# ilur98/DLMC-QUANT

Measured on NVIDIA B200. Metric: fakequant_fwd_bwd_hbm_gbps, higher is better.
Workload: dtype f32

## Files before the change

dlmc_quant_b200/csrc/fq_kernels.cu:

```cuda
#include <mutex>

#include "fq_rows.cuh"

namespace dlmcq {

constexpr int kUnroll = 4;

template <int FORM, typename T, int U = kUnroll, int MINB = 4, bool TILED = false>
__global__ void __launch_bounds__(kThreads, MINB)
fq_fwd_flat(const T* __restrict__ x, T* __restrict__ y, T* __restrict__ codes, int64_t n,
            const float* __restrict__ scale, const float* __restrict__ offset, float g, float lo, float hi,
            int independent) {
  using V = Vec<T>;
  using raw = typename V::raw;
  const int64_t nvec = n / V::N;
  const raw* xv = reinterpret_cast<const raw*>(x);
  const int64_t tile_vecs = static_cast<int64_t>(U) * blockDim.x;
  const int64_t ntiles = nvec / tile_vecs;
  ChanParams p;
  raw r0[U];
  const bool hoist = TILED && independent && blockIdx.x < ntiles;
  if (TILED && independent) {
    p = make_params<FORM>(scale, offset, 0, g, lo, hi);
    if (hoist) {
      const int64_t b = static_cast<int64_t>(blockIdx.x) * tile_vecs + threadIdx.x;
#pragma unroll
      for (int k = 0; k < U; ++k) r0[k] = ld_stream(xv + b + k * blockDim.x);
    }
  }
  pdl_wait();
  pdl_trigger();
  if (!(TILED && independent)) p = make_params<FORM>(scale, offset, 0, g, lo, hi);
  const int64_t stride = static_cast<int64_t>(gridDim.x) * blockDim.x;
  int64_t i = static_cast<int64_t>(blockIdx.x) * blockDim.x + threadIdx.x;
  raw* yv = reinterpret_cast<raw*>(y);
  raw* cv = reinterpret_cast<raw*>(codes);

  auto body = [&](const raw& r, int64_t idx) {
    float f[V::N], fy[V::N], fc[V::N];
// ... 53 lines not shown
    if (codes) codes[i] = from_f32<T>(c);
  }
}

template <int FORM>
__device__ __forceinline__ void finalize_flat(float* partials, int nblocks, float g, float* dscale, float* doffset,
                                              float* smem) {
  double s = 0.0, o = 0.0;
  for (int b = threadIdx.x; b < nblocks; b += blockDim.x) {
    s += static_cast<double>(partials[2 * b]);
    o += static_cast<double>(partials[2 * b + 1]);
  }
  s = warp_sum(s);
  o = warp_sum(o);
  double* sm = reinterpret_cast<double*>(smem);
  const int lane = threadIdx.x & 31, warp = threadIdx.x >> 5, nwarp = blockDim.x >> 5;
  __syncthreads();
  if (lane == 0) { sm[warp] = s; sm[32 + warp] = o; }
  __syncthreads();
  if (threadIdx.x == 0) {
    double ts = 0.0, to = 0.0;
    for (int w = 0; w < nwarp; ++w) { ts += sm[w]; to += sm[32 + w]; }
    float r = static_cast<float>(ts);
    if (FORM == DLMCQ_FORM_AFFINE || FORM == DLMCQ_FORM_A1) r = r * g;
    dscale[0] = r;
    if (doffset) doffset[0] = static_cast<float>(to);
  }
}

template <int FORM, typename T, bool VECTOR, bool WANT_OFF, bool DEFER>
__global__ void __launch_bounds__(kThreads, 4)
fq_bwd_flat(const T* __restrict__ x, const T* __restrict__ dy, T* __restrict__ dx, int64_t n,
            const float* __restrict__ scale, const float* __restrict__ offset, float g, float lo, float hi,
            float* __restrict__ dscale, float* __restrict__ doffset, void* ws, int independent) {
  using V = Vec<T>;
  using raw = typename V::raw;
  __shared__ __align__(16) float smem[128];
  const int64_t nvec = n / V::N;
  const raw* xv = reinterpret_cast<const raw*>(x);
  const raw* gv = reinterpret_cast<const raw*>(dy);
  const int64_t tile_vecs = static_cast<int64_t>(kUnroll) * blockDim.x;
  const int64_t ntiles = nvec / tile_vecs;
  ChanParams p;
  raw rx0[kUnroll], rg0[kUnroll];
  const bool hoist = VECTOR && independent && blockIdx.x < ntiles;
  if (VECTOR && independent) {
    p = make_params<FORM>(scale, offset, 0, g, lo, hi);
    if (hoist) {
      const int64_t b = static_cast<int64_t>(blockIdx.x) * tile_vecs + threadIdx.x;
#pragma unroll
      for (int k = 0; k < kUnroll; ++k) {
        rx0[k] = ld_stream(xv + b + k * blockDim.x);
        rg0[k] = ld_stream(gv + b + k * blockDim.x);
      }
    }
  }
  pdl_wait();
  pdl_trigger();
  if (!(VECTOR && independent)) p = make_params<FORM>(scale, offset, 0, g, lo, hi);
  float acc[2] = {0.f, 0.f};
  const int64_t stride = static_cast<int64_t>(gridDim.x) * blockDim.x;
  int64_t i = static_cast<int64_t>(blockIdx.x) * blockDim.x + threadIdx.x;
  if (VECTOR) {
    raw* ov = reinterpret_cast<raw*>(dx);
    auto body = [&](const raw& rx, const raw& rg, int64_t idx) {
      float fx[V::N], fg[V::N], fo[V::N];
      V::unpack(rx, fx);
      V::unpack(rg, fg);
      fq_vec_bwd<FORM, WANT_OFF, V::N>(fx, fg, p, lo, hi, fo, acc[0], acc[1]);
      st_stream(ov + idx, V::pack(fo));
    };
    int64_t t = blockIdx.x;
    if (hoist) {
      const int64_t b = t * tile_vecs + threadIdx.x;
#pragma unroll
      for (int k = 0; k < kUnroll; ++k) body(rx0[k], rg0[k], b + k * blockDim.x);
      t += gridDim.x;
    }
    for (; t < ntiles; t += gridDim.x) {
      const int64_t b = t * tile_vecs + threadIdx.x;
      raw rx[kUnroll], rg[kUnroll];
#pragma unroll
      for (int k = 0; k < kUnroll; ++k) {
        rx[k] = ld_stream(xv + b + k * blockDim.x);
        rg[k] = ld_stream(gv + b + k * blockDim.x);
      }
#pragma unroll
      for (int k = 0; k < kUnroll; ++k) body(rx[k], rg[k], b + k * blockDim.x);
    }
    for (int64_t j = ntiles * tile_vecs + i; j < nvec; j += stride) body(ld_stream(xv + j), ld_stream(gv + j), j);
    if (blockIdx.x == 0) {
      const int64_t t = nvec * V::N + threadIdx.x;
      if (t < n) dx[t] = from_f32<T>(fq_elem_bwd<FORM, WANT_OFF>(to_f32<T>(x[t]), to_f32<T>(dy[t]), p, lo, hi, acc[0], acc[1]));
    }
  } else {
    for (; i < n; i += stride)
      dx[i] = from_f32<T>(fq_elem_bwd<FORM, WANT_OFF>(to_f32<T>(x[i]), to_f32<T>(dy[i]), p, lo, hi, acc[0], acc[1]));
  }
  block_sum<2>(acc, smem);
  if (DEFER) {
    float* out = static_cast<float*>(ws);
    if (threadIdx.x == 0) {
      if (blockIdx.x == 0) {
        out[0] = __int_as_float(static_cast<int>(gridDim.x));
        out[1] = (FORM == DLMCQ_FORM_AFFINE || FORM == DLMCQ_FORM_A1) ? g : 1.f;
      }
      out[2 + 2 * blockIdx.x] = acc[0];
      out[3 + 2 * blockIdx.x] = acc[1];
    }
    return;
  }
  float* partials = ws_partials(ws);
  if (threadIdx.x == 0) {
    partials[2 * blockIdx.x] = acc[0];
    partials[2 * blockIdx.x + 1] = acc[1];
  }
  if (take_last_ticket(ws_counter(ws), gridDim.x)) {
    finalize_flat<FORM>(partials, gridDim.x, g, dscale, doffset, smem);
    if (threadIdx.x == 0) *ws_counter(ws) = 0u;
  }
}

template <int FORM, typename T>
__global__ void __launch_bounds__(kRowWarps * 32, 3)
fq_fwd_rows(const T* __restrict__ x, T* __restrict__ y, T* __restrict__ codes, RowGeom gm,
            const float* __restrict__ scale, const float* __restrict__ offset, float g, float lo, float hi) {
  const int lane = threadIdx.x & 31;
  const int64_t item = static_cast<int64_t>(blockIdx.x) * kRowWarps + (threadIdx.x >> 5);
  if (item >= gm.rows * gm.segs) return;
  const int64_t row = item / gm.segs, seg = item - row * gm.segs;
// ... 456 lines not shown
    fq_slab_kernel<FORM, T><<<static_cast<unsigned>(sg.groups) * sg.chunks, kThreads, 0, st>>>(
        static_cast<const T*>(x), static_cast<T*>(y), static_cast<T*>(codes), sg, qp->scale, qp->offset, qp->g, lo, hi);
  } else if (cmaj_ok(l->outer, l->channels, l->inner)) {
    const bool vec = cmaj_vec_ok<T>(l->inner, x, y, codes, nullptr);
    const CmajGeom cg = make_cmaj(l->outer, l->channels, l->inner, vec ? Vec<T>::N : 1);
    const int64_t blocks = (cg.channels * cg.chunks + kRowWarps - 1) / kRowWarps;
    if (blocks > 0x7fffffffLL) return DLMCQ_EUNSUPPORTED;
    auto kern = vec ? fq_cmaj_kernel<FORM, T, false, Vec<T>::N> : fq_cmaj_kernel<FORM, T, false, 1>;
    kern<<<static_cast<unsigned>(blocks), kRowWarps * 32, 0, st>>>(
        static_cast<const T*>(x), nullptr, static_cast<T*>(y), static_cast<T*>(codes), cg, qp->scale, qp->offset,
        qp->g, lo, hi, nullptr, nullptr, 0);
  } else {
    const RowGeom gm = make_geom(l);
    const int64_t items = gm.rows * gm.segs;
    const int64_t blocks = (items + kRowWarps - 1) / kRowWarps;
    if (blocks > 0x7fffffffLL) return DLMCQ_EUNSUPPORTED;
    fq_fwd_rows<FORM, T><<<static_cast<unsigned>(blocks), kRowWarps * 32, 0, st>>>(
        static_cast<const T*>(x), static_cast<T*>(y), static_cast<T*>(codes), gm, qp->scale, qp->offset, qp->g, lo, hi);
  }
  DLMCQ_LAUNCH_CHECK();
  return DLMCQ_OK;
}

template <int FORM, typename T>
static int launch_bwd(const void* x, const void* dy, void* dx, float* dscale, float* doffset, const dlmcq_layout* l,
                      const dlmcq_qparams* qp, void* ws, size_t ws_bytes, cudaStream_t st, bool defer = false) {
  const int64_t n = l->outer * l->channels * l->inner;
  const float lo = static_cast<float>(qp->lo), hi = static_cast<float>(qp->hi);
  if (!defer && ws_bytes < dlmcq_workspace_bytes(l)) return DLMCQ_EWORKSPACE;
  if (defer && l->channels != 1) return DLMCQ_EUNSUPPORTED;
  if (l->channels == 1) {
    const bool vec = aligned16(x) && aligned16(dy) && aligned16(dx);
    const int64_t per = vec ? Vec<T>::N : 1;
    int64_t tiles = (n / per + kThreads * kUnroll - 1) / (kThreads * kUnroll);
    int64_t cap = n < (int64_t(1) << 25) ? 888 : (n < (int64_t(1) << 27) ? 2048 : 4096);
    if (cap > kMaxPartialBlocks) cap = kMaxPartialBlocks;
    const int grid = static_cast<int>(tiles < 1 ? 1 : (tiles < cap ? tiles : cap));
    auto k = vec ? (doffset ? fq_bwd_flat<FORM, T, true, true, false> : fq_bwd_flat<FORM, T, true, false, false>)
                 : (doffset ? fq_bwd_flat<FORM, T, false, true, false> : fq_bwd_flat<FORM, T, false, false, false>);
    if (defer) k = vec ? fq_bwd_flat<FORM, T, true, false, true> : fq_bwd_flat<FORM, T, false, false, true>;
    FlatAccess acc;
    if (vec) {
      const size_t bytes = static_cast<size_t>(n) * sizeof(T);
      acc.read(x, bytes);
      acc.read(dy, bytes);
      acc.read(qp->scale, sizeof(float));
      acc.read(qp->offset, sizeof(float));
      if (!defer) acc.read(ws, ws_bytes);
      acc.write(dx, bytes);
      acc.write(dscale, sizeof(float));
      acc.write(doffset, sizeof(float));
      acc.write(ws, defer ? (2 + 2 * static_cast<size_t>(grid)) * sizeof(float) : ws_bytes);
    }
    const int independent = vec ? capture_check(st, acc) : 0;
    cudaError_t e = launch_pdl(k, dim3(grid), dim3(kThreads), 0, st, static_cast<const T*>(x),
                               static_cast<const T*>(dy), static_cast<T*>(dx), n, qp->scale, qp->offset, qp->g, lo, hi,
                               dscale, doffset, ws, independent);
    if (e != cudaSuccess) return set_cuda_error(e);
    if (vec) capture_record(st, acc, independent);
  } else if (doffset == nullptr && n > 0 && tiled_ok<T>(l, x, dy, dx)) {
    const TileGeom tg = make_tile_geom<T>(l);
    const int64_t tiles = (tg.nvec + kTileVecs - 1) / kTileVecs;
    if (tiles > 0x7fffffffLL) return DLMCQ_EUNSUPPORTED;
    fq_tiled_chan_kernel<FORM, T, true><<<static_cast<unsigned>(tiles), kThreads, 0, st>>>(
        static_cast<const T*>(x), static_cast<const T*>(dy), static_cast<T*>(dx), nullptr, tg, qp->scale, qp->offset,
        qp->g, lo, hi, ws_partials(ws));
    DLMCQ_LAUNCH_CHECK();
    const float gmul = (FORM == DLMCQ_FORM_AFFINE || FORM == DLMCQ_FORM_A1) ? qp->g : 1.f;
    tiled_chan_finalize<<<static_cast<unsigned>(l->channels), 128, 0, st>>>(ws_partials(ws), tg, l->outer, gmul, dscale);
  } else if (cmaj_ok(l->outer, l->channels, l->inner) && doffset == nullptr && n > 0) {
    const bool vec = cmaj_vec_ok<T>(l->inner, x, dy, dx, nullptr);
    const CmajGeom cg = make_cmaj(l->outer, l->channels, l->inner, vec ? Vec<T>::N : 1);
    const int64_t blocks = (cg.channels * cg.chunks + kRowWarps - 1) / kRowWarps;
    if (blocks > 0x7fffffffLL) return DLMCQ_EUNSUPPORTED;
    const int direct = cg.chunks == 1 ? 1 : 0;
    auto kern = vec ? fq_cmaj_kernel<FORM, T, true, Vec<T>::N> : fq_cmaj_kernel<FORM, T, true, 1>;
    kern<<<static_cast<unsigned>(blocks), kRowWarps * 32, 0, st>>>(
        static_cast<const T*>(x), static_cast<const T*>(dy), static_cast<T*>(dx), nullptr, cg, qp->scale, qp->offset,
        qp->g, lo, hi, dscale, ws_partials(ws), direct);
    if (!direct) {
      DLMCQ_LAUNCH_CHECK();
      const float gmul = (FORM == DLMCQ_FORM_AFFINE || FORM == DLMCQ_FORM_A1) ? qp->g : 1.f;
      chan_finalize<1><<<static_cast<unsigned>(cg.channels), 128, 0, st>>>(ws_partials(ws), cg.chunks, cg.chunks, 0,
                                                                           gmul, dscale, nullptr);
    }
  } else {
    const RowGeom gm = make_geom(l);
    const int64_t items = gm.rows * gm.segs;
    const int64_t blocks = (items + kRowWarps - 1) / kRowWarps;
    if (blocks > 0x7fffffffLL) return DLMCQ_EUNSUPPORTED;
// ... 8 lines not shown
      chan_finalize<2><<<static_cast<unsigned>(gm.channels), 128, 0, st>>>(
          ws_partials(ws), l->outer * gm.segs, gm.segs, gm.channels * gm.segs, gmul, dscale, doffset);
    }
  }
  DLMCQ_LAUNCH_CHECK();
  return DLMCQ_OK;
}

template <typename T>
static int dispatch_fwd(const void* x, void* y, void* codes, const dlmcq_layout* l, const dlmcq_qparams* qp,
                        cudaStream_t st) {
  switch (qp->form) {
    case DLMCQ_FORM_A1: return launch_fwd<DLMCQ_FORM_A1, T>(x, y, codes, l, qp, st);
    case DLMCQ_FORM_AFFINE: return launch_fwd<DLMCQ_FORM_AFFINE, T>(x, y, codes, l, qp, st);
    case DLMCQ_FORM_ZP: return launch_fwd<DLMCQ_FORM_ZP, T>(x, y, codes, l, qp, st);
    case DLMCQ_FORM_SYM: return launch_fwd<DLMCQ_FORM_SYM, T>(x, y, codes, l, qp, st);
  }
  return DLMCQ_EINVAL;
}
template <typename T>
static int dispatch_bwd(const void* x, const void* dy, void* dx, float* ds, float* doff, const dlmcq_layout* l,
                        const dlmcq_qparams* qp, void* ws, size_t wsb, cudaStream_t st, bool defer = false) {
  switch (qp->form) {
    case DLMCQ_FORM_A1: return launch_bwd<DLMCQ_FORM_A1, T>(x, dy, dx, ds, doff, l, qp, ws, wsb, st, defer);
    case DLMCQ_FORM_AFFINE: return launch_bwd<DLMCQ_FORM_AFFINE, T>(x, dy, dx, ds, doff, l, qp, ws, wsb, st, defer);
    case DLMCQ_FORM_ZP: return launch_bwd<DLMCQ_FORM_ZP, T>(x, dy, dx, ds, doff, l, qp, ws, wsb, st, defer);
    case DLMCQ_FORM_SYM: return launch_bwd<DLMCQ_FORM_SYM, T>(x, dy, dx, ds, doff, l, qp, ws, wsb, st, defer);
  }
  return DLMCQ_EINVAL;
}

__global__ void __launch_bounds__(kThreads)
finalize_many_kernel(const dlmcq_finalize_item* __restrict__ items, int n_items) {
  __shared__ double sm[2][kThreads / 32];
  pdl_wait();
  pdl_trigger();
  const dlmcq_finalize_item it = items[blockIdx.x];
  const float* p = it.partials;
  const int nblocks = __float_as_int(p[0]);
  const float gmul = p[1];
  double s = 0.0, o = 0.0;
  for (int b = threadIdx.x; b < nblocks; b += blockDim.x) {
    s += static_cast<double>(p[2 + 2 * b]);
    o += static_cast<double>(p[3 + 2 * b]);
  }
  s = warp_sum(s);
  o = warp_sum(o);
  const int lane = threadIdx.x & 31, warp = threadIdx.x >> 5;
  if (lane == 0) { sm[0][warp] = s; sm[1][warp] = o; }
  __syncthreads();
  if (threadIdx.x == 0) {
    double ts = 0.0, to = 0.0;
    for (int w = 0; w < kThreads / 32; ++w) { ts += sm[0][w]; to += sm[1][w]; }
    it.dscale[0] = static_cast<float>(ts) * gmul;
    (void)to;
  }
}

}

using namespace dlmcq;

extern "C" size_t dlmcq_workspace_bytes(const dlmcq_layout* l) {
  size_t bytes = kWsHeaderBytes + static_cast<size_t>(kMaxPartialBlocks) * 96 * sizeof(float);
  if (l && l->outer >= 1 && l->channels >= 1 && l->inner >= 0) {
    const RowGeom gm = make_geom(l->outer, l->channels, l->inner);
    const size_t rows_bytes = static_cast<size_t>(gm.rows * gm.segs) * 4 * sizeof(float);
    if (kWsHeaderBytes + rows_bytes > bytes) bytes = kWsHeaderBytes + rows_bytes;
    const size_t tiles = static_cast<size_t>(l->outer * l->channels * l->inner) / (kTileVecs * 4) + 1;
    const size_t tiled_bytes = tiles * kTileRows * sizeof(float);
    if (kWsHeaderBytes + tiled_bytes > bytes) bytes = kWsHeaderBytes + tiled_bytes;
  }
  return bytes;
}

extern "C" int dlmcq_fq_forward(const void* x, void* y, void* codes, const dlmcq_layout* layout,
                                const dlmcq_qparams* qp, void* stream) {
  if (int e = check_layout(layout)) return e;
  if (layout->outer * layout->channels * layout->inner == 0) return DLMCQ_OK;
  if (!qp || !qp->scale || !x || (!y && !codes)) return DLMCQ_EINVAL;
  if (!elem_aligned(x, layout->dtype) || !elem_aligned(y, layout->dtype) || !elem_aligned(codes, layout->dtype))
    return DLMCQ_EALIGN;
  cudaStream_t st = static_cast<cudaStream_t>(stream);
  return layout->dtype == DLMCQ_F32 ? dispatch_fwd<float>(x, y, codes, layout, qp, st)
                                    : dispatch_fwd<__nv_bfloat16>(x, y, codes, layout, qp, st);
}

extern "C" int dlmcq_fq_backward(const void* x, const void* dy, void* dx, float* dscale, float* doffset,
// ... 62 lines not shown
```

dlmc_quant_b200/csrc/grouped_kernels.cu:

```cuda
#include "fq_rows.cuh"

namespace dlmcq {

__device__ __forceinline__ int find_item(const int64_t* __restrict__ prefix, int n_items, int64_t unit) {
  int lo = 0, hi = n_items;
  while (hi - lo > 1) {
    const int mid = (lo + hi) >> 1;
    if (__ldg(prefix + mid) <= unit) lo = mid; else hi = mid;
  }
  return lo;
}

template <int FORM>
__device__ __forceinline__ ChanParams item_params(const dlmcq_group_item& it, int64_t ch) {
  return make_params<FORM>(it.scale, it.offset, ch, it.g, static_cast<float>(it.lo), static_cast<float>(it.hi));
}

template <typename T>
__global__ void __launch_bounds__(kRowWarps * 32)
grouped_fwd_kernel(const dlmcq_group_item* __restrict__ items, const int64_t* __restrict__ prefix, int n_items,
                   int64_t total_units) {
  pdl_wait();
  pdl_trigger();
  const int lane = threadIdx.x & 31;
  const int64_t unit = static_cast<int64_t>(blockIdx.x) * kRowWarps + (threadIdx.x >> 5);
  if (unit >= total_units) return;
  const int k = find_item(prefix, n_items, unit);
  const dlmcq_group_item it = items[k];
  const int64_t local = unit - __ldg(prefix + k);
  const int64_t segs = (it.inner + DLMCQ_GROUP_SEG - 1) / DLMCQ_GROUP_SEG;
  const int64_t row = local / segs, seg = local - row * segs;
  const int64_t beg = seg * DLMCQ_GROUP_SEG;
  const int64_t len = (it.inner - beg) < DLMCQ_GROUP_SEG ? (it.inner - beg) : DLMCQ_GROUP_SEG;
  const T* xr = static_cast<const T*>(it.x) + row * it.inner + beg;
  T* yr = static_cast<T*>(it.y) + row * it.inner + beg;
  const float lo = static_cast<float>(it.lo), hi = static_cast<float>(it.hi);
  switch (it.form) {
    case DLMCQ_FORM_A1: fwd_row_segment<DLMCQ_FORM_A1, T>(xr, yr, nullptr, len, item_params<DLMCQ_FORM_A1>(it, row), lo, hi, lane); break;
    case DLMCQ_FORM_AFFINE: fwd_row_segment<DLMCQ_FORM_AFFINE, T>(xr, yr, nullptr, len, item_params<DLMCQ_FORM_AFFINE>(it, row), lo, hi, lane); break;
    case DLMCQ_FORM_ZP: fwd_row_segment<DLMCQ_FORM_ZP, T>(xr, yr, nullptr, len, item_params<DLMCQ_FORM_ZP>(it, row), lo, hi, lane); break;
    default: fwd_row_segment<DLMCQ_FORM_SYM, T>(xr, yr, nullptr, len, item_params<DLMCQ_FORM_SYM>(it, row), lo, hi, lane); break;
  }
}

template <typename T>
__global__ void __launch_bounds__(kRowWarps * 32)
grouped_bwd_kernel(const dlmcq_group_item* __restrict__ items, const int64_t* __restrict__ prefix, int n_items,
                   int64_t total_units, float* __restrict__ partials) {
  pdl_wait();
  pdl_trigger();
  const int lane = threadIdx.x & 31;
  const int64_t unit = static_cast<int64_t>(blockIdx.x) * kRowWarps + (threadIdx.x >> 5);
  if (unit >= total_units) return;
  const int k = find_item(prefix, n_items, unit);
  const dlmcq_group_item it = items[k];
  const int64_t local = unit - __ldg(prefix + k);
  const int64_t segs = (it.inner + DLMCQ_GROUP_SEG - 1) / DLMCQ_GROUP_SEG;
  const int64_t row = local / segs, seg = local - row * segs;
  const int64_t beg = seg * DLMCQ_GROUP_SEG;
  const int64_t len = (it.inner - beg) < DLMCQ_GROUP_SEG ? (it.inner - beg) : DLMCQ_GROUP_SEG;
  const int64_t base = row * it.inner + beg;
  const T* xr = static_cast<const T*>(it.x) + base;
  const T* gr = static_cast<const T*>(it.dy) + base;
  T* dr = static_cast<T*>(it.y) + base;
  const float lo = static_cast<float>(it.lo), hi = static_cast<float>(it.hi);
  float as = 0.f, ao = 0.f;
  switch (it.form) {
    case DLMCQ_FORM_A1: bwd_row_segment<DLMCQ_FORM_A1, T>(xr, gr, dr, len, item_params<DLMCQ_FORM_A1>(it, row), lo, hi, lane, as, ao); break;
    case DLMCQ_FORM_AFFINE: bwd_row_segment<DLMCQ_FORM_AFFINE, T>(xr, gr, dr, len, item_params<DLMCQ_FORM_AFFINE>(it, row), lo, hi, lane, as, ao); break;
    case DLMCQ_FORM_ZP: bwd_row_segment<DLMCQ_FORM_ZP, T>(xr, gr, dr, len, item_params<DLMCQ_FORM_ZP>(it, row), lo, hi, lane, as, ao); break;
    default: bwd_row_segment<DLMCQ_FORM_SYM, T>(xr, gr, dr, len, item_params<DLMCQ_FORM_SYM>(it, row), lo, hi, lane, as, ao); break;
  }
  if (lane == 0) partials[unit] = as;
}

__global__ void __launch_bounds__(kRowWarps * 32)
grouped_finalize_kernel(const dlmcq_group_item* __restrict__ items, const int64_t* __restrict__ prefix,
                        const int64_t* __restrict__ chan_prefix, int n_items, int64_t total_channels,
                        const float* __restrict__ partials) {
  pdl_wait();
  pdl_trigger();
  const int lane = threadIdx.x & 31;
  const int64_t gch = static_cast<int64_t>(blockIdx.x) * kRowWarps + (threadIdx.x >> 5);
  if (gch >= total_channels) return;
  const int k = find_item(chan_prefix, n_items, gch);
  const dlmcq_group_item it = items[k];
  const int64_t ch = gch - __ldg(chan_prefix + k);
  const int64_t segs = (it.inner + DLMCQ_GROUP_SEG - 1) / DLMCQ_GROUP_SEG;
  const float* p = partials + __ldg(prefix + k) + ch * segs;
  double s = 0.0;
  for (int64_t j = lane; j < segs; j += 32) s += static_cast<double>(p[j]);
  s = warp_sum(s);
  if (lane == 0) {
    float r = static_cast<float>(s);
    if (it.form == DLMCQ_FORM_AFFINE || it.form == DLMCQ_FORM_A1) r = r * it.g;
    it.dscale[ch] = r;
  }
}

}

using namespace dlmcq;

extern "C" int dlmcq_fq_forward_grouped(const dlmcq_group_item* items, const int64_t* unit_prefix, int n_items,
                                        int64_t total_units, int dtype, void* stream) {
  if (!items || !unit_prefix || n_items < 1 || total_units < 0) return DLMCQ_EINVAL;
  if (total_units == 0) return DLMCQ_OK;
  const int64_t blocks = (total_units + kRowWarps - 1) / kRowWarps;
  if (blocks > 0x7fffffffLL) return DLMCQ_EUNSUPPORTED;
  cudaStream_t st = static_cast<cudaStream_t>(stream);
  if (dtype != DLMCQ_F32 && dtype != DLMCQ_BF16) return DLMCQ_EINVAL;
  cudaError_t e = launch_pdl(dtype == DLMCQ_F32 ? grouped_fwd_kernel<float> : grouped_fwd_kernel<__nv_bfloat16>,
                             dim3(static_cast<unsigned>(blocks)), dim3(kRowWarps * 32), 0, st, items, unit_prefix,
                             n_items, total_units);
  if (e != cudaSuccess) return set_cuda_error(e);
  return DLMCQ_OK;
}

extern "C" int dlmcq_fq_backward_grouped(const dlmcq_group_item* items, const int64_t* unit_prefix,
                                         const int64_t* chan_prefix, int n_items, int64_t total_units,
                                         int64_t total_channels, int dtype, float* partials, void* stream) {
  if (!items || !unit_prefix || !chan_prefix || !partials || n_items < 1 || total_units < 0) return DLMCQ_EINVAL;
  if (total_units == 0) return DLMCQ_OK;
  const int64_t blocks = (total_units + kRowWarps - 1) / kRowWarps;
  const int64_t fblocks = (total_channels + kRowWarps - 1) / kRowWarps;
  if (blocks > 0x7fffffffLL || fblocks > 0x7fffffffLL) return DLMCQ_EUNSUPPORTED;
  cudaStream_t st = static_cast<cudaStream_t>(stream);
  if (dtype != DLMCQ_F32 && dtype != DLMCQ_BF16) return DLMCQ_EINVAL;
  cudaError_t e = launch_pdl(dtype == DLMCQ_F32 ? grouped_bwd_kernel<float> : grouped_bwd_kernel<__nv_bfloat16>,
                             dim3(static_cast<unsigned>(blocks)), dim3(kRowWarps * 32), 0, st, items, unit_prefix,
                             n_items, total_units, partials);
  if (e != cudaSuccess) return set_cuda_error(e);
  e = launch_pdl(grouped_finalize_kernel, dim3(static_cast<unsigned>(fblocks)), dim3(kRowWarps * 32), 0, st, items,
                 unit_prefix, chan_prefix, n_items, total_channels, partials);
  if (e != cudaSuccess) return set_cuda_error(e);
  return DLMCQ_OK;
}
```

Before: 6566.

## Reschedule flat backward tiles with contiguous chunks or fixed-grid striding

Changes the flat backward kernel's work assignment. Large inputs now get one block per contiguous chunk of tiles instead of a capped grid-stride loop, mid-size inputs use a fixed 888-block stride, and small inputs get one tile per block. The goal is better load balance and locality across SMs, at the cost of more partials per launch and a more complex tail condition. The finalize kernel also drops its unused offset accumulation and unrolls its partial loads, and a sweep script is added to compare schedules.

```diff
diff --git a/dlmc_quant_b200/csrc/fq_kernels.cu b/dlmc_quant_b200/csrc/fq_kernels.cu
--- a/dlmc_quant_b200/csrc/fq_kernels.cu
+++ b/dlmc_quant_b200/csrc/fq_kernels.cu
@@ -5,6 +5,8 @@
 namespace dlmcq {
 
 constexpr int kUnroll = 4;
+constexpr int64_t kBwdStrideTiles = 3136;
+constexpr int64_t kBwdStrideGrid = 888;
 
 template <int FORM, typename T, int U = kUnroll, int MINB = 4, bool TILED = false>
 __global__ void __launch_bounds__(kThreads, MINB)
@@ -124,70 +126,65 @@
 __global__ void __launch_bounds__(kThreads, 4)
 fq_bwd_flat(const T* __restrict__ x, const T* __restrict__ dy, T* __restrict__ dx, int64_t n,
             const float* __restrict__ scale, const float* __restrict__ offset, float g, float lo, float hi,
-            float* __restrict__ dscale, float* __restrict__ doffset, void* ws, int independent) {
+            float* __restrict__ dscale, float* __restrict__ doffset, void* ws, int64_t first, int64_t step, int64_t count, int independent) {
   using V = Vec<T>;
   using raw = typename V::raw;
   __shared__ __align__(16) float smem[128];
   const int64_t nvec = n / V::N;
   const raw* xv = reinterpret_cast<const raw*>(x);
   const raw* gv = reinterpret_cast<const raw*>(dy);
-  const int64_t tile_vecs = static_cast<int64_t>(kUnroll) * blockDim.x;
+  const int64_t tile_vecs = static_cast<int64_t>(kUnroll) * kThreads;
   const int64_t ntiles = nvec / tile_vecs;
+  const int64_t t0 = static_cast<int64_t>(blockIdx.x) * first;
   ChanParams p;
-  raw rx0[kUnroll], rg0[kUnroll];
-  const bool hoist = VECTOR && independent && blockIdx.x < ntiles;
+  raw rx[kUnroll], rg[kUnroll];
+  auto load = [&](int64_t t) {
+    const int64_t b = t * tile_vecs + threadIdx.x;
+#pragma unroll
+    for (int k = 0; k < kUnroll; ++k) {
+      rx[k] = ld_stream(xv + b + k * kThreads);
+      rg[k] = ld_stream(gv + b + k * kThreads);
+    }
+  };
+  const bool hoist = VECTOR && independent && t0 < ntiles;
   if (VECTOR && independent) {
     p = make_params<FORM>(scale, offset, 0, g, lo, hi);
-    if (hoist) {
-      const int64_t b = static_cast<int64_t>(blockIdx.x) * tile_vecs + threadIdx.x;
-#pragma unroll
-      for (int k = 0; k < kUnroll; ++k) {
-        rx0[k] = ld_stream(xv + b + k * blockDim.x);
-        rg0[k] = ld_stream(gv + b + k * blockDim.x);
-      }
-    }
+    if (hoist) load(t0);
   }
   pdl_wait();
   pdl_trigger();
   if (!(VECTOR && independent)) p = make_params<FORM>(scale, offset, 0, g, lo, hi);
   float acc[2] = {0.f, 0.f};
-  const int64_t stride = static_cast<int64_t>(gridDim.x) * blockDim.x;
-  int64_t i = static_cast<int64_t>(blockIdx.x) * blockDim.x + threadIdx.x;
   if (VECTOR) {
     raw* ov = reinterpret_cast<raw*>(dx);
-    auto body = [&](const raw& rx, const raw& rg, int64_t idx) {
+    auto body = [&](const raw& r, const raw& q, int64_t idx) {
       float fx[V::N], fg[V::N], fo[V::N];
-      V::unpack(rx, fx);
-      V::unpack(rg, fg);
+      V::unpack(r, fx);
+      V::unpack(q, fg);
       fq_vec_bwd<FORM, WANT_OFF, V::N>(fx, fg, p, lo, hi, fo, acc[0], acc[1]);
       st_stream(ov + idx, V::pack(fo));
     };
-    int64_t t = blockIdx.x;
-    if (hoist) {
+    int64_t t = t0;
+    for (int64_t k = 0; k < count && t < ntiles; ++k, t += step) {
+      if (k != 0 || !hoist) load(t);
       const int64_t b = t * tile_vecs + threadIdx.x;
 #pragma unroll
-      for (int k = 0; k < kUnroll; ++k) body(rx0[k], rg0[k], b + k * blockDim.x);
-      t += gridDim.x;
-    }
-    for (; t < ntiles; t += gridDim.x) {
-      const int64_t b = t * tile_vecs + threadIdx.x;
-      raw rx[kUnroll], rg[kUnroll];
-#pragma unroll
-      for (int k = 0; k < kUnroll; ++k) {
-        rx[k] = ld_stream(xv + b + k * blockDim.x);
-        rg[k] = ld_stream(gv + b + k * blockDim.x);
-      }
-#pragma unroll
-      for (int k = 0; k < kUnroll; ++k) body(rx[k], rg[k], b + k * blockDim.x);
-    }
-    for (int64_t j = ntiles * tile_vecs + i; j < nvec; j += stride) body(ld_stream(xv + j), ld_stream(gv + j), j);
+      for (int k = 0; k < kUnroll; ++k) body(rx[k], rg[k], b + k * kThreads);
+    }
+    if (ntiles >= t0 && (ntiles - t0) % step == 0 && (ntiles - t0) / step < count)
+      for (int64_t j = ntiles * tile_vecs + threadIdx.x; j < nvec; j += kThreads)
+        body(ld_stream(xv + j), ld_stream(gv + j), j);
     if (blockIdx.x == 0) {
-      const int64_t t = nvec * V::N + threadIdx.x;
-      if (t < n) dx[t] = from_f32<T>(fq_elem_bwd<FORM, WANT_OFF>(to_f32<T>(x[t]), to_f32<T>(dy[t]), p, lo, hi, acc[0], acc[1]));
+      const int64_t e = nvec * V::N + threadIdx.x;
+      if (e < n) dx[e] = from_f32<T>(fq_elem_bwd<FORM, WANT_OFF>(to_f32<T>(x[e]), to_f32<T>(dy[e]), p, lo, hi, acc[0], acc[1]));
     }
   } else {
-    for (; i < n; i += stride)
-      dx[i] = from_f32<T>(fq_elem_bwd<FORM, WANT_OFF>(to_f32<T>(x[i]), to_f32<T>(dy[i]), p, lo, hi, acc[0], acc[1]));
+    int64_t t = t0;
+    for (int64_t k = 0; k < count && t * tile_vecs < n; ++k, t += step) {
+      const int64_t end = (t + 1) * tile_vecs < n ? (t + 1) * tile_vecs : n;
+      for (int64_t i = t * tile_vecs + threadIdx.x; i < end; i += kThreads)
+        dx[i] = from_f32<T>(fq_elem_bwd<FORM, WANT_OFF>(to_f32<T>(x[i]), to_f32<T>(dy[i]), p, lo, hi, acc[0], acc[1]));
+    }
   }
   block_sum<2>(acc, smem);
   if (DEFER) {
@@ -710,10 +707,16 @@
   if (l->channels == 1) {
     const bool vec = aligned16(x) && aligned16(dy) && aligned16(dx);
     const int64_t per = vec ? Vec<T>::N : 1;
-    int64_t tiles = (n / per + kThreads * kUnroll - 1) / (kThreads * kUnroll);
-    int64_t cap = n < (int64_t(1) << 25) ? 888 : (n < (int64_t(1) << 27) ? 2048 : 4096);
-    if (cap > kMaxPartialBlocks) cap = kMaxPartialBlocks;
-    const int grid = static_cast<int>(tiles < 1 ? 1 : (tiles < cap ? tiles : cap));
+    const int64_t tiles = (n / per + kThreads * kUnroll - 1) / (kThreads * kUnroll);
+    int64_t first = 1, step = 1, count = 1, blocks = tiles < 1 ? 1 : tiles;
+    if (tiles > kBwdStrideTiles) {
+      first = count = tiles > kMaxPartialBlocks ? (tiles + kMaxPartialBlocks - 1) / kMaxPartialBlocks : 1;
+      blocks = (tiles + first - 1) / first;
+    } else if (tiles > kBwdStrideGrid) {
+      step = blocks = kBwdStrideGrid;
+      count = (tiles + kBwdStrideGrid - 1) / kBwdStrideGrid;
+    }
+    const int grid = static_cast<int>(blocks);
     auto k = vec ? (doffset ? fq_bwd_flat<FORM, T, true, true, false> : fq_bwd_flat<FORM, T, true, false, false>)
                  : (doffset ? fq_bwd_flat<FORM, T, false, true, false> : fq_bwd_flat<FORM, T, false, false, false>);
     if (defer) k = vec ? fq_bwd_flat<FORM, T, true, false, true> : fq_bwd_flat<FORM, T, false, false, true>;
@@ -733,7 +736,7 @@
     const int independent = vec ? capture_check(st, acc) : 0;
     cudaError_t e = launch_pdl(k, dim3(grid), dim3(kThreads), 0, st, static_cast<const T*>(x),
                                static_cast<const T*>(dy), static_cast<T*>(dx), n, qp->scale, qp->offset, qp->g, lo, hi,
-                               dscale, doffset, ws, independent);
+                               dscale, doffset, ws, first, step, count, independent);
     if (e != cudaSuccess) return set_cuda_error(e);
     if (vec) capture_record(st, acc, independent);
   } else if (doffset == nullptr && n > 0 && tiled_ok<T>(l, x, dy, dx)) {
@@ -808,28 +811,31 @@
 
 __global__ void __launch_bounds__(kThreads)
 finalize_many_kernel(const dlmcq_finalize_item* __restrict__ items, int n_items) {
-  __shared__ double sm[2][kThreads / 32];
+  __shared__ double sm[kThreads / 32];
   pdl_wait();
   pdl_trigger();
   const dlmcq_finalize_item it = items[blockIdx.x];
   const float* p = it.partials;
   const int nblocks = __float_as_int(p[0]);
   const float gmul = p[1];
-  double s = 0.0, o = 0.0;
-  for (int b = threadIdx.x; b < nblocks; b += blockDim.x) {
-    s += static_cast<double>(p[2 + 2 * b]);
-    o += static_cast<double>(p[3 + 2 * b]);
-  }
+  double s = 0.0;
+  int b = threadIdx.x;
+  for (; b + 3 * kThreads < nblocks; b += 4 * kThreads) {
+    float v[4];
+#pragma unroll
+    for (int k = 0; k < 4; ++k) v[k] = p[2 + 2 * (b + k * kThreads)];
+#pragma unroll
+    for (int k = 0; k < 4; ++k) s += static_cast<double>(v[k]);
+  }
+  for (; b < nblocks; b += kThreads) s += static_cast<double>(p[2 + 2 * b]);
   s = warp_sum(s);
-  o = warp_sum(o);
   const int lane = threadIdx.x & 31, warp = threadIdx.x >> 5;
-  if (lane == 0) { sm[0][warp] = s; sm[1][warp] = o; }
+  if (lane == 0) sm[warp] = s;
   __syncthreads();
   if (threadIdx.x == 0) {
-    double ts = 0.0, to = 0.0;
-    for (int w = 0; w < kThreads / 32; ++w) { ts += sm[0][w]; to += sm[1][w]; }
+    double ts = 0.0;
+    for (int w = 0; w < kThreads / 32; ++w) ts += sm[w];
     it.dscale[0] = static_cast<float>(ts) * gmul;
-    (void)to;
   }
 }
 
diff --git a/profiles/bwd_schedule_sweep.py b/profiles/bwd_schedule_sweep.py
--- /dev/null
+++ b/profiles/bwd_schedule_sweep.py
@@ -0,0 +1,126 @@
+import argparse
+import ctypes as C
+import json
+import math
+import os
+import statistics
+import subprocess
+import sys
+
+ROOT = os.path.dirname(os.path.dirname(os.path.abspath(__file__)))
+if ROOT not in sys.path:
+    sys.path.insert(0, ROOT)
+
+SIZES = [3211264, 6422528, 12845056, 19267584, 25690112, 51380224, 1 << 26, 102760448]
+MIN_FOOTPRINT = 512 << 20
+
+
+def card():
+    import torch
+    info = {"gpu": torch.cuda.get_device_name()}
+    try:
+        q = subprocess.run(["nvidia-smi", "--query-gpu=name,power.limit,clocks.max.sm", "--format=csv,noheader",
+                            "-i", str(torch.cuda.current_device())], capture_output=True, text=True, timeout=30)
+        name, power, clock = [s.strip() for s in q.stdout.strip().split(",")]
+        info.update(smi_name=name, power_limit=power, max_sm_clock=clock)
+    except Exception as e:
+        info["smi_error"] = repr(e)
+    return info
+
+
+def load(path):
+    from dlmc_quant_b200 import _lib
+    h = C.CDLL(os.path.abspath(path))
+    for name in ("dlmcq_fq_backward_partials", "dlmcq_fq_partials_floats", "dlmcq_status_string"):
+        fn = getattr(h, name)
+        fn.restype, fn.argtypes = _lib.SIGNATURES[name]
+    return h
+
+
+def main():
+    ap = argparse.ArgumentParser()
+    ap.add_argument("--lib", action="append", default=[], metavar="LABEL=PATH")
+    ap.add_argument("--sizes", default=",".join(map(str, SIZES)))
+    ap.add_argument("--dtypes", default="f32,bf16")
+    ap.add_argument("--rounds", type=int, default=5)
+    ap.add_argument("--out", default=None)
+    args = ap.parse_args()
+    import torch
+    from dlmc_quant_b200 import _lib
+
+    libs = [(s.split("=", 1)[0], load(s.split("=", 1)[1])) for s in args.lib] or [("tree", load(_lib.LIB_PATH))]
+    out = open(args.out, "w") if args.out else None
+
+    def emit(rec):
+        print(json.dumps(rec), flush=True)
+        if out:
+            out.write(json.dumps(rec) + "\n")
+
+    emit(card())
+    dev = torch.device("cuda")
+    floats = libs[0][1].dlmcq_fq_partials_floats()
+    for dt in args.dtypes.split(","):
+        tdt, ldt, esz = (torch.float32, _lib.F32, 4) if dt == "f32" else (torch.bfloat16, _lib.BF16, 2)
+        for n in map(int, args.sizes.split(",")):
+            nbuf = max(4, min(16, math.ceil(MIN_FOOTPRINT / (3 * esz * n))))
+            gen = torch.Generator(device=dev).manual_seed(n)
+            xs = [(torch.relu(torch.randn(n, generator=gen, device=dev)) * 2).to(tdt) for _ in range(nbuf)]
+            dys = [torch.randn(n, generator=gen, device=dev).to(tdt) for _ in range(nbuf)]
+            dxs = [torch.empty(n, dtype=tdt, device=dev) for _ in range(nbuf)]
+            scale = torch.tensor([6.0 / 15], device=dev)
+            off = torch.zeros(1, device=dev)
+            qp = _lib.QParams(_lib.FORM_AFFINE, 0, 15, 1 / math.sqrt(n * 15), scale.data_ptr(), off.data_ptr())
+            lay = _lib.Layout(1, 1, n, ldt)
+            parts = torch.empty(nbuf, floats, device=dev)
+
+            def chain(h):
+                st = C.c_void_p(torch.cuda.current_stream().cuda_stream)
+                for i in range(nbuf):
+                    rc = h.dlmcq_fq_backward_partials(xs[i].data_ptr(), dys[i].data_ptr(), dxs[i].data_ptr(),
+                                                      C.byref(lay), C.byref(qp), parts[i].data_ptr(), st)
+                    if rc:
+                        raise RuntimeError(h.dlmcq_status_string(rc).decode())
+
+            graphs, ref = [], None
+            for label, h in libs:
+                chain(h)
+                torch.cuda.synchronize()
+                g = torch.cuda.CUDAGraph()
+                with torch.cuda.graph(g):
+                    chain(h)
+                for d in dxs:
+                    d.fill_(float("nan"))
+                g.replay()
+                torch.cuda.synchronize()
+                if ref is None:
+                    ref = dxs[0].view(torch.int16 if esz == 2 else torch.int32).clone()
+                elif not torch.equal(ref, dxs[0].view(ref.dtype)):
+                    raise SystemExit(f"{label}: dx differs from {libs[0][0]} at n={n} {dt}")
+                graphs.append(g)
+            per_replay = nbuf * 3 * esz * n / 6.5e12
+            replays = max(3, math.ceil(0.03 / per_replay))
+            times = [[] for _ in libs]
+            e0, e1 = torch.cuda.Event(enable_timing=True), torch.cuda.Event(enable_timing=True)
+            for g in graphs:
+                g.replay()
+            for _ in range(args.rounds):
+                for k, g in enumerate(graphs):
+                    g.replay()
+                    e0.record()
+                    for _ in range(replays):
+                        g.replay()
+                    e1.record()
+                    e1.synchronize()
+                    times[k].append(e0.elapsed_time(e1) * 1e3 / (replays * nbuf))
+            for (label, _), ts in zip(libs, times):
+                us = statistics.median(ts)
+                emit({"lib": label, "dtype": dt, "n": n, "tiles": math.ceil(n * esz / 16 / 1024), "launches": nbuf,
+                      "replays": replays, "us_per_launch": round(us, 3),
+                      "spread_us": round(max(ts) - min(ts), 3),
+                      "gbps": round(3 * esz * n / (us * 1e-6) / 1e9, 1)})
+            del graphs, xs, dys, dxs, parts
+            torch.cuda.empty_cache()
+
+
+if __name__ == "__main__":
+    main()
```

After: 6646 (median of 6 runs). 1.2% higher.

## Pipeline grouped fake-quant segments with unrolled streaming loads and warp-parallel item search

Applied to the files above, without the earlier changes.

Replaces the per-warp binary search with a ballot-based 32-way warp search. Adds custom forward and backward segment loops that prefetch several vectors ahead with streaming loads and stores, and sets minimum-blocks launch bounds. Backward walks blocks in reverse order and writes dscale directly when a row has a single segment. The finalize kernel becomes a per-item 2D grid that exits early for single-segment items. These changes target latency and wasted finalize work, at the cost of more registers and more complex code.

```diff
diff --git a/dlmc_quant_b200/csrc/grouped_kernels.cu b/dlmc_quant_b200/csrc/grouped_kernels.cu
--- a/dlmc_quant_b200/csrc/grouped_kernels.cu
+++ b/dlmc_quant_b200/csrc/grouped_kernels.cu
@@ -2,99 +2,218 @@
 
 namespace dlmcq {
 
-__device__ __forceinline__ int find_item(const int64_t* __restrict__ prefix, int n_items, int64_t unit) {
+constexpr int kGroupFwdUnroll = 8;
+template <typename T>
+constexpr int group_bwd_unroll() { return sizeof(T) == 4 ? 4 : 3; }
+
+__device__ __forceinline__ int find_item_warp(const int64_t* __restrict__ prefix, int n_items, int64_t unit,
+                                              int lane) {
   int lo = 0, hi = n_items;
   while (hi - lo > 1) {
-    const int mid = (lo + hi) >> 1;
-    if (__ldg(prefix + mid) <= unit) lo = mid; else hi = mid;
+    const int step = (hi - lo + 31) >> 5;
+    const int idx = lo + lane * step;
+    const bool le = idx < hi && __ldg(prefix + idx) <= unit;
+    const unsigned m = __ballot_sync(0xffffffffu, le);
+    lo += (31 - __clz(m)) * step;
+    hi = min(hi, lo + step);
   }
   return lo;
 }
 
-template <int FORM>
-__device__ __forceinline__ ChanParams item_params(const dlmcq_group_item& it, int64_t ch) {
-  return make_params<FORM>(it.scale, it.offset, ch, it.g, static_cast<float>(it.lo), static_cast<float>(it.hi));
+struct UnitPos {
+  dlmcq_group_item it;
+  int64_t row, beg, len, segs;
+};
+__device__ __forceinline__ UnitPos locate_unit(const dlmcq_group_item* __restrict__ items,
+                                               const int64_t* __restrict__ prefix, int n_items, int64_t unit,
+                                               int lane) {
+  UnitPos u;
+  const int k = find_item_warp(prefix, n_items, unit, lane);
+  u.it = items[k];
+  const int64_t local = unit - __ldg(prefix + k);
+  u.segs = (u.it.inner + DLMCQ_GROUP_SEG - 1) / DLMCQ_GROUP_SEG;
+  int64_t seg = 0;
+  u.row = local;
+  if (u.segs > 1) {
+    u.row = local / u.segs;
+    seg = local - u.row * u.segs;
+  }
+  u.beg = seg * DLMCQ_GROUP_SEG;
+  u.len = (u.it.inner - u.beg) < DLMCQ_GROUP_SEG ? (u.it.inner - u.beg) : DLMCQ_GROUP_SEG;
+  return u;
+}
+
+template <int FORM, typename T>
+__device__ __forceinline__ void fwd_segment(const T* __restrict__ xr, T* __restrict__ yr, int64_t len,
+                                            const dlmcq_group_item& it, int64_t row, int lane) {
+  using V = Vec<T>;
+  using raw = typename V::raw;
+  constexpr int U = kGroupFwdUnroll;
+  const float lo = static_cast<float>(it.lo), hi = static_cast<float>(it.hi);
+  const bool vec_ok = ((reinterpret_cast<uintptr_t>(xr) | reinterpret_cast<uintptr_t>(yr)) & 15u) == 0;
+  const int nvec = vec_ok ? static_cast<int>(len) / V::N : 0;
+  const raw* xv = reinterpret_cast<const raw*>(xr);
+  raw* yv = reinterpret_cast<raw*>(yr);
+  raw r[U];
+  int j = lane;
+#pragma unroll
+  for (int h = 0; h < U; ++h)
+    if (j + 32 * h < nvec) r[h] = ld_stream(xv + j + 32 * h);
+  const ChanParams p = make_params<FORM>(it.scale, it.offset, row, it.g, lo, hi);
+  while (true) {
+#pragma unroll
+    for (int h = 0; h < U; ++h) {
+      if (j + 32 * h < nvec) {
+        float f[V::N], fy[V::N], fc[V::N];
+        V::unpack(r[h], f);
+        fq_vec<FORM, V::N>(f, p, lo, hi, fc, fy);
+        st_stream(yv + j + 32 * h, V::pack(fy));
+      }
+    }
+    j += 32 * U;
+    if (j >= nvec) break;
+#pragma unroll
+    for (int h = 0; h < U; ++h)
+      if (j + 32 * h < nvec) r[h] = ld_stream(xv + j + 32 * h);
+  }
+  for (int e = nvec * V::N + lane; e < len; e += 32) {
+    float c, v;
+    fq_elem<FORM>(to_f32<T>(xr[e]), p, lo, hi, c, v);
+    yr[e] = from_f32<T>(v);
+  }
+}
+
+template <int FORM, typename T>
+__device__ __forceinline__ float bwd_segment(const T* __restrict__ xr, const T* __restrict__ gr, T* __restrict__ dr,
+                                             int64_t len, const dlmcq_group_item& it, int64_t row, int lane) {
+  using V = Vec<T>;
+  using raw = typename V::raw;
+  constexpr int U = group_bwd_unroll<T>();
+  const float lo = static_cast<float>(it.lo), hi = static_cast<float>(it.hi);
+  const bool vec_ok = ((reinterpret_cast<uintptr_t>(xr) | reinterpret_cast<uintptr_t>(gr) |
+                        reinterpret_cast<uintptr_t>(dr)) & 15u) == 0;
+  const int nvec = vec_ok ? static_cast<int>(len) / V::N : 0;
+  const raw* xv = reinterpret_cast<const raw*>(xr);
+  const raw* gv = reinterpret_cast<const raw*>(gr);
+  raw* dv = reinterpret_cast<raw*>(dr);
+  raw rx[U], rg[U];
+  int j = lane;
+#pragma unroll
+  for (int h = 0; h < U; ++h) {
+    if (j + 32 * h < nvec) {
+      rx[h] = ld_stream(xv + j + 32 * h);
+      rg[h] = ld_stream(gv + j + 32 * h);
+    }
+  }
+  const ChanParams p = make_params<FORM>(it.scale, it.offset, row, it.g, lo, hi);
+  float as = 0.f, ao = 0.f;
+  while (j < nvec) {
+#pragma unroll
+    for (int h = 0; h < U; ++h) {
+      if (j + 32 * h < nvec) {
+        float fx[V::N], fg[V::N], fo[V::N];
+        V::unpack(rx[h], fx);
+        V::unpack(rg[h], fg);
+        fq_vec_bwd<FORM, true, V::N>(fx, fg, p, lo, hi, fo, as, ao);
+        st_stream(dv + j + 32 * h, V::pack(fo));
+      }
+    }
+    j += 32 * U;
+    if (j >= nvec) break;
+#pragma unroll
+    for (int h = 0; h < U; ++h) {
+      if (j + 32 * h < nvec) {
+        rx[h] = ld_stream(xv + j + 32 * h);
+        rg[h] = ld_stream(gv + j + 32 * h);
+      }
+    }
+  }
+  for (int e = nvec * V::N + lane; e < len; e += 32)
+    dr[e] = from_f32<T>(fq_elem_bwd<FORM, true>(to_f32<T>(xr[e]), to_f32<T>(gr[e]), p, lo, hi, as, ao));
+  return warp_sum(as);
+}
+
+template <bool FROM_END>
+__device__ __forceinline__ int64_t unit_of_warp() {
+  const int64_t b = FROM_END ? gridDim.x - 1 - blockIdx.x : blockIdx.x;
+  return b * kRowWarps + (threadIdx.x >> 5);
 }
 
 template <typename T>
-__global__ void __launch_bounds__(kRowWarps * 32)
+__global__ void __launch_bounds__(kRowWarps * 32, 4)
 grouped_fwd_kernel(const dlmcq_group_item* __restrict__ items, const int64_t* __restrict__ prefix, int n_items,
                    int64_t total_units) {
   pdl_wait();
   pdl_trigger();
   const int lane = threadIdx.x & 31;
-  const int64_t unit = static_cast<int64_t>(blockIdx.x) * kRowWarps + (threadIdx.x >> 5);
+  const int64_t unit = unit_of_warp<false>();
   if (unit >= total_units) return;
-  const int k = find_item(prefix, n_items, unit);
-  const dlmcq_group_item it = items[k];
-  const int64_t local = unit - __ldg(prefix + k);
-  const int64_t segs = (it.inner + DLMCQ_GROUP_SEG - 1) / DLMCQ_GROUP_SEG;
-  const int64_t row = local / segs, seg = local - row * segs;
-  const int64_t beg = seg * DLMCQ_GROUP_SEG;
-  const int64_t len = (it.inner - beg) < DLMCQ_GROUP_SEG ? (it.inner - beg) : DLMCQ_GROUP_SEG;
-  const T* xr = static_cast<const T*>(it.x) + row * it.inner + beg;
-  T* yr = static_cast<T*>(it.y) + row * it.inner + beg;
-  const float lo = static_cast<float>(it.lo), hi = static_cast<float>(it.hi);
-  switch (it.form) {
-    case DLMCQ_FORM_A1: fwd_row_segment<DLMCQ_FORM_A1, T>(xr, yr, nullptr, len, item_params<DLMCQ_FORM_A1>(it, row), lo, hi, lane); break;
-    case DLMCQ_FORM_AFFINE: fwd_row_segment<DLMCQ_FORM_AFFINE, T>(xr, yr, nullptr, len, item_params<DLMCQ_FORM_AFFINE>(it, row), lo, hi, lane); break;
-    case DLMCQ_FORM_ZP: fwd_row_segment<DLMCQ_FORM_ZP, T>(xr, yr, nullptr, len, item_params<DLMCQ_FORM_ZP>(it, row), lo, hi, lane); break;
-    default: fwd_row_segment<DLMCQ_FORM_SYM, T>(xr, yr, nullptr, len, item_params<DLMCQ_FORM_SYM>(it, row), lo, hi, lane); break;
+  const UnitPos u = locate_unit(items, prefix, n_items, unit, lane);
+  const int64_t base = u.row * u.it.inner + u.beg;
+  const T* xr = static_cast<const T*>(u.it.x) + base;
+  T* yr = static_cast<T*>(u.it.y) + base;
+  switch (u.it.form) {
+    case DLMCQ_FORM_A1: fwd_segment<DLMCQ_FORM_A1, T>(xr, yr, u.len, u.it, u.row, lane); break;
+    case DLMCQ_FORM_AFFINE: fwd_segment<DLMCQ_FORM_AFFINE, T>(xr, yr, u.len, u.it, u.row, lane); break;
+    case DLMCQ_FORM_ZP: fwd_segment<DLMCQ_FORM_ZP, T>(xr, yr, u.len, u.it, u.row, lane); break;
+    default: fwd_segment<DLMCQ_FORM_SYM, T>(xr, yr, u.len, u.it, u.row, lane); break;
   }
 }
 
 template <typename T>
-__global__ void __launch_bounds__(kRowWarps * 32)
+__global__ void __launch_bounds__(kRowWarps * 32, sizeof(T) == 4 ? 4 : 3)
 grouped_bwd_kernel(const dlmcq_group_item* __restrict__ items, const int64_t* __restrict__ prefix, int n_items,
                    int64_t total_units, float* __restrict__ partials) {
   pdl_wait();
   pdl_trigger();
   const int lane = threadIdx.x & 31;
-  const int64_t unit = static_cast<int64_t>(blockIdx.x) * kRowWarps + (threadIdx.x >> 5);
+  const int64_t unit = unit_of_warp<true>();
   if (unit >= total_units) return;
-  const int k = find_item(prefix, n_items, unit);
-  const dlmcq_group_item it = items[k];
-  const int64_t local = unit - __ldg(prefix + k);
-  const int64_t segs = (it.inner + DLMCQ_GROUP_SEG - 1) / DLMCQ_GROUP_SEG;
-  const int64_t row = local / segs, seg = local - row * segs;
-  const int64_t beg = seg * DLMCQ_GROUP_SEG;
-  const int64_t len = (it.inner - beg) < DLMCQ_GROUP_SEG ? (it.inner - beg) : DLMCQ_GROUP_SEG;
-  const int64_t base = row * it.inner + beg;
-  const T* xr = static_cast<const T*>(it.x) + base;
-  const T* gr = static_cast<const T*>(it.dy) + base;
-  T* dr = static_cast<T*>(it.y) + base;
-  const float lo = static_cast<float>(it.lo), hi = static_cast<float>(it.hi);
-  float as = 0.f, ao = 0.f;
-  switch (it.form) {
-    case DLMCQ_FORM_A1: bwd_row_segment<DLMCQ_FORM_A1, T>(xr, gr, dr, len, item_params<DLMCQ_FORM_A1>(it, row), lo, hi, lane, as, ao); break;
-    case DLMCQ_FORM_AFFINE: bwd_row_segment<DLMCQ_FORM_AFFINE, T>(xr, gr, dr, len, item_params<DLMCQ_FORM_AFFINE>(it, row), lo, hi, lane, as, ao); break;
-    case DLMCQ_FORM_ZP: bwd_row_segment<DLMCQ_FORM_ZP, T>(xr, gr, dr, len, item_params<DLMCQ_FORM_ZP>(it, row), lo, hi, lane, as, ao); break;
-    default: bwd_row_segment<DLMCQ_FORM_SYM, T>(xr, gr, dr, len, item_params<DLMCQ_FORM_SYM>(it, row), lo, hi, lane, as, ao); break;
-  }
-  if (lane == 0) partials[unit] = as;
-}
-
+  const UnitPos u = locate_unit(items, prefix, n_items, unit, lane);
+  const int64_t base = u.row * u.it.inner + u.beg;
+  const T* xr = static_cast<const T*>(u.it.x) + base;
+  const T* gr = static_cast<const T*>(u.it.dy) + base;
+  T* dr = static_cast<T*>(u.it.y) + base;
+  float as;
+  switch (u.it.form) {
+    case DLMCQ_FORM_A1: as = bwd_segment<DLMCQ_FORM_A1, T>(xr, gr, dr, u.len, u.it, u.row, lane); break;
+    case DLMCQ_FORM_AFFINE: as = bwd_segment<DLMCQ_FORM_AFFINE, T>(xr, gr, dr, u.len, u.it, u.row, lane); break;
+    case DLMCQ_FORM_ZP: as = bwd_segment<DLMCQ_FORM_ZP, T>(xr, gr, dr, u.len, u.it, u.row, lane); break;
+    default: as = bwd_segment<DLMCQ_FORM_SYM, T>(xr, gr, dr, u.len, u.it, u.row, lane); break;
+  }
+  if (lane == 0) {
+    if (u.segs == 1) {
+      u.it.dscale[u.row] = (u.it.form == DLMCQ_FORM_AFFINE || u.it.form == DLMCQ_FORM_A1) ? as * u.it.g : as;
+    } else {
+      partials[unit] = as;
+    }
+  }
+}
+
+constexpr int kFinalizeSlices = 64;
 __global__ void __launch_bounds__(kRowWarps * 32)
 grouped_finalize_kernel(const dlmcq_group_item* __restrict__ items, const int64_t* __restrict__ prefix,
-                        const int64_t* __restrict__ chan_prefix, int n_items, int64_t total_channels,
                         const float* __restrict__ partials) {
   pdl_wait();
   pdl_trigger();
+  const int k = blockIdx.x;
+  const int64_t inner = items[k].inner;
+  const int64_t segs = (inner + DLMCQ_GROUP_SEG - 1) / DLMCQ_GROUP_SEG;
+  if (segs == 1) return;
+  const dlmcq_group_item it = items[k];
   const int lane = threadIdx.x & 31;
-  const int64_t gch = static_cast<int64_t>(blockIdx.x) * kRowWarps + (threadIdx.x >> 5);
-  if (gch >= total_channels) return;
-  const int k = find_item(chan_prefix, n_items, gch);
-  const dlmcq_group_item it = items[k];
-  const int64_t ch = gch - __ldg(chan_prefix + k);
-  const int64_t segs = (it.inner + DLMCQ_GROUP_SEG - 1) / DLMCQ_GROUP_SEG;
-  const float* p = partials + __ldg(prefix + k) + ch * segs;
-  double s = 0.0;
-  for (int64_t j = lane; j < segs; j += 32) s += static_cast<double>(p[j]);
-  s = warp_sum(s);
-  if (lane == 0) {
-    float r = static_cast<float>(s);
-    if (it.form == DLMCQ_FORM_AFFINE || it.form == DLMCQ_FORM_A1) r = r * it.g;
-    it.dscale[ch] = r;
+  const float* pk = partials + __ldg(prefix + k);
+  const int64_t stride = static_cast<int64_t>(gridDim.y) * kRowWarps;
+  for (int64_t ch = static_cast<int64_t>(blockIdx.y) * kRowWarps + (threadIdx.x >> 5); ch < it.channels; ch += stride) {
+    const float* p = pk + ch * segs;
+    double s = 0.0;
+    for (int64_t j = lane; j < segs; j += 32) s += static_cast<double>(p[j]);
+    s = warp_sum(s);
+    if (lane == 0) {
+      float r = static_cast<float>(s);
+      if (it.form == DLMCQ_FORM_AFFINE || it.form == DLMCQ_FORM_A1) r = r * it.g;
+      it.dscale[ch] = r;
+    }
   }
 }
 
@@ -131,8 +250,8 @@
                              dim3(static_cast<unsigned>(blocks)), dim3(kRowWarps * 32), 0, st, items, unit_prefix,
                              n_items, total_units, partials);
   if (e != cudaSuccess) return set_cuda_error(e);
-  e = launch_pdl(grouped_finalize_kernel, dim3(static_cast<unsigned>(fblocks)), dim3(kRowWarps * 32), 0, st, items,
-                 unit_prefix, chan_prefix, n_items, total_channels, partials);
+  e = launch_pdl(grouped_finalize_kernel, dim3(static_cast<unsigned>(n_items), kFinalizeSlices), dim3(kRowWarps * 32), 0, st, items,
+                 unit_prefix, static_cast<const float*>(partials));
   if (e != cudaSuccess) return set_cuda_error(e);
   return DLMCQ_OK;
 }
diff --git a/profiles/prof_grouped.py b/profiles/prof_grouped.py
--- /dev/null
+++ b/profiles/prof_grouped.py
@@ -0,0 +1,114 @@
+import argparse
+import json
+import math
+import os
+import statistics
+import sys
+
+ROOT = os.path.dirname(os.path.dirname(os.path.abspath(__file__)))
+if ROOT not in sys.path:
+    sys.path.insert(0, ROOT)
+
+
+def make_entries(layers, dtype, gen):
+    import torch
+    from dlmc_quant_b200 import _lib
+    from dlmc_quant_b200 import functional as F
+    lo, hi = -7, 7
+    fwd, bwd = [], []
+    for shape in layers:
+        c, k = shape[0], math.prod(shape[1:])
+        w = torch.randn((c, k), generator=gen, device="cuda") * 0.02
+        scale, _ = F.minmax_from_stats(F.obs_stats(w, ch_axis=0), 4, True)
+        x = w.to(dtype)
+        dy = torch.randn((c, k), generator=gen, device="cuda").to(dtype)
+        e = dict(x=x, dy=dy, y=torch.empty_like(x), scale=scale, offset=None, dscale=torch.empty(c, device="cuda"),
+                 channels=c, inner=k, form=_lib.FORM_AFFINE, lo=lo, hi=hi, g=1 / math.sqrt(c * k * hi))
+        fwd.append(e)
+        bwd.append(dict(e, y=torch.empty_like(x)))
+    return fwd, bwd
+
+
+def graph_us(fn, iters, reps):
+    import torch
+    fn()
+    torch.cuda.synchronize()
+    g = torch.cuda.CUDAGraph()
+    with torch.cuda.graph(g):
+        for _ in range(iters):
+            fn()
+    g.replay()
+    torch.cuda.synchronize()
+    times = []
+    for _ in range(reps):
+        a, b = torch.cuda.Event(enable_timing=True), torch.cuda.Event(enable_timing=True)
+        a.record()
+        g.replay()
+        b.record()
+        torch.cuda.synchronize()
+        times.append(a.elapsed_time(b) * 1e3 / iters)
+    return statistics.median(times), min(times), max(times)
+
+
+def main():
+    ap = argparse.ArgumentParser()
+    ap.add_argument("--iters", type=int, default=50)
+    ap.add_argument("--reps", type=int, default=5)
+    ap.add_argument("--out", default=None)
+    args = ap.parse_args()
+    import torch
+    from dlmc_quant_b200 import functional as F
+
+    import bench
+    shapes = [w for _, _, w in bench.resnet50_layers()]
+    inner = lambda s: math.prod(s[1:])
+    tables = {"full": shapes, "short": [s for s in shapes if inner(s) <= 512],
+              "long": [s for s in shapes if inner(s) >= 2048], "reversed": shapes[::-1]}
+    rows = []
+    head = {"gpu": torch.cuda.get_device_name(), "iters": args.iters, "reps": args.reps}
+    print(json.dumps(head), flush=True)
+
+    def emit(row):
+        rows.append(row)
+        print(json.dumps(row), flush=True)
+
+    for dtype in (torch.float32, torch.bfloat16):
+        esz = torch.finfo(dtype).bits // 8
+        for name, table in tables.items():
+            gen = torch.Generator(device="cuda").manual_seed(2333)
+            fwd, bwd = make_entries(table, dtype, gen)
+            n = sum(e["x"].numel() for e in fwd)
+            units = sum(e["channels"] * -(-e["inner"] // F.GROUP_SEG) for e in fwd)
+            gf, gb = F.GroupedFakeQuant("cuda"), F.GroupedFakeQuant("cuda")
+            f = graph_us(lambda: gf.forward(fwd, dtype), args.iters, args.reps)
+            b = graph_us(lambda: gb.backward(bwd, dtype), args.iters, args.reps)
+            emit({"table": name, "dtype": str(dtype).split(".")[-1], "tensors": len(fwd), "elements": n, "units": units,
+                  "fwd_us": round(f[0], 2), "fwd_us_min_max": [round(f[1], 2), round(f[2], 2)],
+                  "fwd_tbps": round(2 * esz * n / f[0] / 1e6, 3),
+                  "bwd_us": round(b[0], 2), "bwd_us_min_max": [round(b[1], 2), round(b[2], 2)],
+                  "bwd_tbps": round(3 * esz * n / b[0] / 1e6, 3)})
+            del fwd, bwd, gf, gb
+        n = sum(math.prod(s) for s in shapes)
+        x = (torch.randn(n, device="cuda") * 0.02).to(dtype)
+        dy = torch.randn(n, device="cuda").to(dtype)
+        y = torch.empty_like(x)
+        scale = torch.full((1,), 0.02 / 7, device="cuda")
+        off = torch.zeros(1, device="cuda")
+        g = 1 / math.sqrt(n * 7)
+        c = graph_us(lambda: y.copy_(x), args.iters, args.reps)
+        ff = graph_us(lambda: F.fq_forward(x, scale, off, -7, 7, F.FORM_AFFINE, g=g), args.iters, args.reps)
+        fb = graph_us(lambda: F.fq_backward(x, dy, scale, off, -7, 7, F.FORM_AFFINE, g=g), args.iters, args.reps)
+        emit({"table": "reference", "dtype": str(dtype).split(".")[-1], "elements": n,
+              "copy_us": round(c[0], 2), "copy_tbps": round(2 * esz * n / c[0] / 1e6, 3),
+              "flat_fwd_us": round(ff[0], 2), "flat_fwd_tbps": round(2 * esz * n / ff[0] / 1e6, 3),
+              "flat_bwd_us": round(fb[0], 2), "flat_bwd_tbps": round(3 * esz * n / fb[0] / 1e6, 3)})
+        del x, dy, y
+        torch.cuda.empty_cache()
+    if args.out:
+        with open(args.out, "w") as fh:
+            for r in [head] + rows:
+                fh.write(json.dumps(r) + "\n")
+
+
+if __name__ == "__main__":
+    main()
```

Measured after the change: 6575 before, 6620 after, median of 6. About the same (+0.7%).
